# soycan-sim/bendy-tracer

Measured on AMD Instinct MI355X. Metric: Msamples/s (pixels x spp / s) at 1080p, higher is better.
Workload: dtype f32; 1 GPU; C3: scene.json.gz 1920x1080x64spp Subsample::None, Config=main.rs (max_bounces 8, max_volume_bounces 32, clip 0.01..1000, volume_step 0.1, Output::Full), flat space (the reference has no lens code), seed 0x5EED; parallelism=single

## Files before the change

### bendy_tracer_amd/api.py

```python
from __future__ import annotations

import ctypes as C
import enum
import os
from dataclasses import dataclass
from typing import Optional

import numpy as np

_HERE = os.path.dirname(os.path.abspath(__file__))
LIB_PATH = os.path.join(_HERE, "libbendy_hip.so")
BT_TILE = 16


class BendyError(RuntimeError):

    def __init__(self, code, message):
        super().__init__(f"[bt_status {code}] {message}")
        self.code = code


class Output(enum.IntEnum):
    Full = 0
    Albedo = 1
# ... 184 lines not shown


class _CLens(C.Structure):
    _fields_ = [("centre", C.c_float * 3), ("rs", C.c_float), ("step", C.c_float), ("radius", C.c_float),
                ("max_steps", C.c_uint32)]


EXPORTS = [
    "bt_config_default", "bt_render_config_default", "bt_last_error", "bt_last_error_code", "bt_version", "bt_scene_load",
    "bt_scene_from_json", "bt_scene_free", "bt_scene_find_by_tag", "bt_scene_set_camera_aspect", "bt_scene_set_lens",
    "bt_scene_object_count", "bt_scene_data_count", "bt_scene_export_prims", "bt_render", "bt_render_device",
    "bt_shard_floats", "bt_render_shard_device", "bt_unshard_device", "bt_preview_device", "bt_preview",
    "bt_comm_unique_id", "bt_comm_init", "bt_comm_free", "bt_comm_rank", "bt_comm_world", "bt_allgather_shards_device",
    "bt_exchange_frame_device", "bt_scene_last_stats", "bt_tuning_default", "bt_scene_set_tuning", "bt_scene_get_tuning", "bt_scene_default", "bt_scene_to_json", "bt_scene_save", "bt_write_png",
    "bt_scene_trim", "bt_denoise_params_default", "bt_denoiser_new", "bt_denoiser_free", "bt_denoise_device",
    "bt_denoise", "bt_debug_primary_mask", "bt_debug_block_masks_device", "bt_debug_mask_key", "bt_debug_set_object",
    "bt_debug_plan_launch",
    "bt_render_guided_device", "bt_adaptive_params_default", "bt_adaptive_new", "bt_adaptive_free", "bt_adaptive_reset",
    "bt_render_adaptive_device", "bt_adaptive_poll", "bt_adaptive_counts", "bt_adaptive_errors", "bt_debug_adaptive_moments",
    "bt_adaptive_resolve_device",
    "bt_scene_camera_view", "bt_scene_set_camera_pose", "bt_temporal_params_default", "bt_temporal_new", "bt_temporal_free",
    "bt_temporal_reset", "bt_temporal_accumulate_device", "bt_debug_temporal_history", "bt_debug_reproject",
    "bt_display_params_default", "bt_display_new", "bt_display_free", "bt_display_reset", "bt_display_device",
    "bt_display_exposure", "bt_debug_display_histogram", "bt_write_pfm", "bt_scene_export_sorted_rows",
    "bt_debug_abs_limit",
    "bt_glare_params_default", "bt_glare_new", "bt_glare_free", "bt_glare_device", "bt_debug_glare_plane", "bt_debug_glare_host",
    "bt_resample_params_default", "bt_resample_new", "bt_resample_free", "bt_resample_device", "bt_debug_resample_weights",
    "bt_debug_resample_plane", "bt_debug_resample_host",
    "bt_despeckle_params_default", "bt_despeckle_new", "bt_despeckle_free", "bt_despeckle_device", "bt_despeckle_poll",
    "bt_debug_despeckle_host",
    "bt_upscale_params_default", "bt_upscale_new", "bt_upscale_free", "bt_upscale_device", "bt_upscale_poll",
# ... 30 lines not shown
    L.bt_scene_find_by_tag.argtypes = [vp, C.c_char_p, C.POINTER(C.c_uint64)]
    L.bt_scene_set_camera_aspect.argtypes = [vp, C.c_uint64, C.c_float]
    L.bt_scene_set_lens.argtypes = [vp, C.POINTER(_CLens)]
    L.bt_scene_object_count.argtypes = [vp]
    L.bt_scene_data_count.argtypes = [vp]
    L.bt_scene_export_prims.argtypes = [vp, fp, C.c_int]
    L.bt_scene_export_sorted_rows.argtypes = [vp, C.POINTER(C.c_uint32), C.c_int]
    L.bt_debug_abs_limit.restype = C.c_float
    L.bt_debug_abs_limit.argtypes = [C.c_float]
    L.bt_debug_primary_mask.argtypes = [vp, C.c_uint64, C.POINTER(_CConfig), C.POINTER(_CRenderConfig), C.c_uint32, C.c_uint32,
                                        C.c_uint32, C.c_uint32, C.c_uint32, C.POINTER(C.c_uint64), C.c_uint32]
    L.bt_debug_set_object.argtypes = [vp, C.c_uint64, fp, C.c_float]
    L.bt_debug_block_masks_device.argtypes = L.bt_debug_primary_mask.argtypes
    L.bt_debug_mask_key.argtypes = [vp, C.c_uint64, C.POINTER(_CConfig), C.POINTER(_CRenderConfig), C.c_uint32, C.c_uint32,
                                    C.c_uint32, C.c_uint32, C.c_uint32, C.POINTER(C.c_uint8), C.c_uint32]
    L.bt_debug_plan_launch.argtypes = [vp, C.c_uint64, C.POINTER(_CConfig), C.POINTER(_CRenderConfig), C.c_uint32, C.c_uint32,
                                       C.c_uint32, C.c_uint32, C.c_int32, C.c_uint32, C.c_int32, C.c_uint32, C.c_uint64,
                                       C.POINTER(Stats)]
    L.bt_render.argtypes = [vp, C.c_uint64, C.POINTER(_CConfig), C.POINTER(_CRenderConfig), fp, C.c_uint32,
                            C.c_uint32, C.c_uint64]
    L.bt_render_device.argtypes = [vp, C.c_uint64, C.POINTER(_CConfig), C.POINTER(_CRenderConfig), vp, C.c_uint32,
                                   C.c_uint32, C.c_uint64, vp]
    L.bt_render_guided_device.argtypes = [vp, C.c_uint64, C.POINTER(_CConfig), C.POINTER(_CRenderConfig), vp, vp, vp, vp,
                                          C.c_uint32, C.c_uint32, C.c_uint64, vp]
    L.bt_shard_floats.restype = C.c_size_t
    L.bt_shard_floats.argtypes = [C.c_uint32, C.c_uint32, C.c_uint32]
    L.bt_render_shard_device.argtypes = [vp, C.c_uint64, C.POINTER(_CConfig), C.POINTER(_CRenderConfig), vp,
                                         C.c_uint32, C.c_uint32, C.c_uint32, C.c_uint32, C.c_uint64, vp]
    L.bt_unshard_device.argtypes = [vp, vp, C.c_uint32, C.c_uint32, C.c_uint32, vp]
    L.bt_preview_device.argtypes = [vp, vp, C.c_uint32, C.c_uint32, C.c_uint32, C.c_int32, vp]
# ... 410 lines not shown
                                             None, 0))
        out = np.zeros(n, dtype=np.uint64)
        _check(lib.bt_debug_primary_mask(scene._h, camera, C.byref(c), C.byref(r), width, height, slices, rank, world,
                                         out.ctypes.data_as(C.POINTER(C.c_uint64)), n))
        return out

    def block_masks_device(self, scene: Scene, camera: int, config: RenderConfig, width, height, slices, rank=0, world=1):
        c, r = _c_configs(self.config, config, 0)
        n = _check(lib.bt_debug_block_masks_device(scene._h, camera, C.byref(c), C.byref(r), width, height, slices, rank,
                                                   world, None, 0))
        out = np.zeros(n, dtype=np.uint64)
        _check(lib.bt_debug_block_masks_device(scene._h, camera, C.byref(c), C.byref(r), width, height, slices, rank, world,
                                               out.ctypes.data_as(C.POINTER(C.c_uint64)), n))
        return out

    def mask_key(self, scene: Scene, camera: int, config: RenderConfig, width, height, slices, rank=0, world=1) -> bytes:
        c, r = _c_configs(self.config, config, 0)
        n = _check(lib.bt_debug_mask_key(scene._h, camera, C.byref(c), C.byref(r), width, height, slices, rank, world, None, 0))
        out = (C.c_uint8 * n)()
        _check(lib.bt_debug_mask_key(scene._h, camera, C.byref(c), C.byref(r), width, height, slices, rank, world, out, n))
        return bytes(out)

    def plan_launch(self, scene: Scene, camera: int, config: RenderConfig, width, height, n_cu, rank=0, world=1, sharded=False,
                    kind=0, guides=0, alloc_limit=0) -> Stats:
        c, r = _c_configs(self.config, config, 0)
        st = Stats()
        _check(lib.bt_debug_plan_launch(scene._h, camera, C.byref(c), C.byref(r), width, height, rank, world, int(sharded),
                                        n_cu, kind, guides, alloc_limit, C.byref(st)))
        return st

# ... 901 lines not shown
```

### bendy_tracer_amd/csrc/bt_api.cpp

```cpp
#include <hip/hip_runtime.h>

#include <algorithm>
#include <cmath>
#include <cstdlib>
#include <cstdio>
#include <cstring>
#include <memory>
#include <string>

#include "../../include/bendy_hip.h"
#include "bt_internal.hpp"
#include "bt_scene.hpp"
#include "bt_types.h"
#include "bt_cull.hpp"
#include "bt_plan.hpp"

#pragma STDC FP_CONTRACT OFF

namespace {

thread_local std::string g_error;
thread_local int g_error_code = 0;
constexpr uint32_t kCounterSlots = 64;

// ... 39 lines not shown
    DeviceArray<BtSphereRow> d_sphere_rows;
    DeviceArray<BtRectAAN> d_aan_rows;
    DeviceArray<BtRectLA> d_la_rows;
    DeviceArray<int32_t> d_other_rows;
    DeviceArray<float> d_density;
    DeviceArray<int32_t> d_lens_prims;
    bt_lens lens_prims_for{};
    bool lens_prims_valid = false;
    unsigned long long *d_counters = nullptr;
    uint32_t render_seq = 0;
    uint32_t last_slot = 0;
    DeviceArray<float> d_scratch;
    uint32_t scratch_small_streak = 0;
    btplan::Scratch plan_scratch;
    DeviceArray<uint64_t> d_block_masks;
    btcull::MaskKey masks_for{};
    uint64_t rows_generation = 0;
    DeviceArray<float> d_host_frame;
    int n_cu = 0;
    bt_tuning tuning{};
    hipEvent_t ev_start = nullptr, ev_stop = nullptr;
    bt_stats last{};
    bool lens_on = false;
    bt_lens lens{};
    bool stats_pending = false;

    bt_scene() { bt_tuning_default(&tuning); }
    void release_device_state() {
        if (d_counters) (void)hipFree(d_counters);
        if (ev_start) (void)hipEventDestroy(ev_start);
        if (ev_stop) (void)hipEventDestroy(ev_stop);
        d_counters = nullptr;
        ev_start = ev_stop = nullptr;
        stats_pending = false;
        release_buffers();
    }
    void release_buffers() {
        d_scratch.release();
        d_host_frame.release();
        d_block_masks.release();
        masks_for = btcull::MaskKey{};
        scratch_small_streak = 0;
    }
    ~bt_scene() { release_device_state(); }
};

namespace {

int ensure_flat(bt_scene *s) {
    if (s->flat_valid) return 0;
    try {
        s->flat = bt::flatten_scene(s->scene);
    } catch (const bt::Error &e) {
        return fail(e.code, e.message);
    }
// ... 214 lines not shown
    if (!s->lens_on) return 0;
    if (!s->lens_prims_valid || std::memcmp(&s->lens_prims_for, &s->lens, sizeof(bt_lens)) != 0) {
        BT_HIP(s->d_lens_prims.upload(lens_candidates(s->flat.prims, s->lens, (double)s->lens.radius + (double)P.lens_margin)));
        s->lens_prims_for = s->lens;
        s->lens_prims_valid = true;
    }
    P.lens_prims = s->d_lens_prims.ptr;
    P.n_lens_prims = (int32_t)s->d_lens_prims.count;
    return 0;
}

int ensure_block_masks(bt_scene *s, BtLaunch &P, uint32_t n_blocks, hipStream_t stream) {
    btcull::MaskKey key;
    btcull::mask_key(key, P, n_blocks, s->rows_generation, (const void *)stream);
    if (!bt_mask_cache_enabled() || std::memcmp(&key, &s->masks_for, sizeof key) != 0) {
        if (s->d_block_masks.count < n_blocks) {
            if (s->d_block_masks.ptr) BT_HIP(hipDeviceSynchronize());
            s->masks_for = btcull::MaskKey{};
            BT_HIP(s->d_block_masks.allocate(n_blocks));
        }
        s->masks_for = btcull::MaskKey{};
        BT_HIP(bt_launch_block_masks(&P, n_blocks, s->d_block_masks.ptr, stream));
        s->masks_for = key;
    }
    P.block_masks = s->d_block_masks.ptr;
    return 0;
}

uint64_t realloc_scratch(bt_scene *s, hipStream_t stream, uint64_t need) {
    if (s->d_scratch.ptr && hipStreamSynchronize(stream) != hipSuccess) return s->d_scratch.bytes();
    s->d_scratch.release();
    if (need && s->d_scratch.allocate(need / sizeof(float)) != hipSuccess) (void)hipGetLastError();
    return s->d_scratch.bytes();
}

struct RenderPass {
    int kind = btplan::PLAIN;
    float *guides[3] = {nullptr, nullptr, nullptr};
    const uint32_t *tile_active = nullptr;
    float *moment = nullptr;
// ... 25 lines not shown
    if (rcode) return fail(rcode, plan.error);
    P.scratch = s->d_scratch.ptr;
    for (int g = 0; g < 3; ++g) {
        P.guide_out[g] = plan.output == 4 ? pass.guides[g] : nullptr;
        P.guide_scratch[g] = plan.guide_values[g] ? P.scratch + plan.guide_values[g] : nullptr;
    }
    P.tile_active = pass.tile_active;
    P.moment = pass.moment;

    s->last_slot = s->render_seq % kCounterSlots;
    if (s->last_slot == 0) BT_HIP(hipMemsetAsync(s->d_counters, 0, kCounterSlots * 16 * sizeof(unsigned long long), stream));
    s->render_seq += 1;
    P.counters = s->d_counters + (size_t)s->last_slot * 16;
    BT_HIP(hipEventRecord(s->ev_start, stream));
    P.block_masks = nullptr;
    if (bt_launch_reads_masks(&P, plan.output)) {
        rcode = ensure_block_masks(s, P, plan.grid * (uint32_t)P.slices, stream);
        if (rcode) return rcode;
    }
    {
        const uint32_t all = (uint32_t)P.samples, base = P.sample_base;
        for (uint32_t done = 0; done < all; done += plan.chunk) {
            P.samples = (int32_t)std::min(plan.chunk, all - done);
            P.sample_base = base + done;
            BT_HIP(bt_launch_render(&P, plan.output, plan.grid, plan.lds_bytes, stream));
        }
        P.samples = (int32_t)all;
        P.sample_base = base;
    }
    BT_HIP(hipEventRecord(s->ev_stop, stream));
// ... 311 lines not shown
    if (n_blocks < 0) return n_blocks;
    if (!masks || cap == 0) return n_blocks;
    if (P.any_rects || P.any_volumes) return fail(BT_ERR_INVALID_ARG, "the scene does not run the build that reads block masks");
    int rc = ensure_device(scene);
    if (rc) return rc;
    n_blocks = debug_mask_launch(scene, camera_ref, config, render, width, height, slices, rank, world, P);
    if (n_blocks < 0) return n_blocks;
    uint64_t *d = nullptr;
    BT_HIP(hipMalloc((void **)&d, sizeof(uint64_t) * (size_t)n_blocks));
    hipError_t e = bt_launch_block_masks(&P, (uint32_t)n_blocks, d, nullptr);
    if (e == hipSuccess)
        e = hipMemcpy(masks, d, sizeof(uint64_t) * (size_t)std::min<uint32_t>(cap, (uint32_t)n_blocks), hipMemcpyDeviceToHost);
    (void)hipFree(d);
    if (e != hipSuccess) return fail(BT_ERR_DEVICE, hipGetErrorString(e));
    return n_blocks;
}

int bt_debug_mask_key(bt_scene *scene, uint64_t camera_ref, const bt_config *config, const bt_render_config *render,
                      uint32_t width, uint32_t height, uint32_t slices, uint32_t rank, uint32_t world, uint8_t *out,
                      uint32_t cap) {
    BtLaunch P;
    const int n_blocks = debug_mask_launch(scene, camera_ref, config, render, width, height, slices, rank, world, P);
    if (n_blocks < 0) return n_blocks;
    btcull::MaskKey key;
    P.sphere_rows = nullptr;
    btcull::mask_key(key, P, (uint32_t)n_blocks, scene->rows_generation, nullptr);
    if (out && cap > 0) std::memcpy(out, &key, std::min<size_t>(cap, sizeof key));
    return (int)sizeof key;
}

// ... 182 lines not shown
```

### bendy_tracer_amd/csrc/bt_cull.hpp

```cpp
#pragma once
#include <stdint.h>
#include <string.h>

#include "bt_types.h"

#if defined(__HIPCC__) || defined(__HIP__)
#define BT_HD __host__ __device__ inline
#define BT_HDF static __host__ __device__ __forceinline__
#else
#define BT_HD inline
#define BT_HDF static inline
#endif

struct BlockGeom { uint32_t NS, LOG_NS, pxb, LOG_PXB, LBW, WMASK; };
BT_HDF BlockGeom block_geom(const BtLaunch &P) {
    BlockGeom g;
    g.NS = (uint32_t)P.slices;
    g.LOG_NS = (uint32_t)__builtin_ctz(g.NS);
    g.pxb = 256u >> g.LOG_NS;
    g.LOG_PXB = 8u - g.LOG_NS;
    g.LBW = g.pxb >= 32 ? 3u : 2u;
    g.WMASK = (1u << g.LBW) - 1u;
    return g;
}
// ... 186 lines not shown

template <class Rows> BT_HD uint64_t block_mask(const BtLaunch &P, Rows rows, uint32_t b) {
    const BlockGeom G = block_geom(P);
    const BlockRef B = block_ref(P, G, b);
    uint32_t nx = 0, ny = 0;
    block_extent(P, G, B, nx, ny);
    if (nx == 0u || ny == 0u || P.n_prims <= 0) return 0ull;
    if (P.n_prims > 64) return ~0ull;
    const Cone K = primary_cone(P, B.px0, B.py0, nx, ny);
    uint64_t m = 0;
    for (int i = 0; i < P.n_prims; ++i)
        if (may_hit(K, rows[i].cx, rows[i].cy, rows[i].cz, rows[i].r2)) m |= 1ull << i;
    return m;
}

struct MaskKey {
    BtV3 cam_cx, cam_cy, cam_cz, cam_t;
    float yfov, xfov, pixel_width, pixel_height;
    float jitter_u_lo, jitter_u_scale, jitter_v_lo, jitter_v_scale;
    int32_t subsample_n, has_focus;
    float focus, aperture;
    BtV3 disk_x, disk_y;
    float one_scale, clip_min;
    uint32_t width, height, tiles_x, tiles_y, tiles_x_magic;
    int32_t slices, sharded;
    uint32_t rank, world;
    int32_t n_prims;
    uint32_t n_blocks;
    uint32_t valid;
    uint64_t rows_generation;
// ... 26 lines not shown
```

### bendy_tracer_amd/csrc/bt_internal.hpp

```cpp
#pragma once
#include <hip/hip_runtime.h>

#include <string>

#include "../../include/bendy_hip.h"
#include "bt_view.hpp"

struct BtLaunch;
struct BtSphereRow;

struct BtTemporalLaunch {
    btview::View cur, prev;
    const float4 *color, *normal, *depth;
    float nc, nn, nd;
    const float4 *hist_in, *guide_in;
    float4 *hist_out, *guide_out, *out;
    float alpha_min, max_history, depth_tolerance, normal_min;
};

#define BT_DISPLAY_BINS 256
#define BT_DISPLAY_COUNTERS 258
#define BT_DISPLAY_STRIDE 260
struct BtDisplayState {
    float e;
// ... 1 lines not shown
    float shown_ev, shown_mult;
};
struct BtDisplayExpose {
    double log2_key;
    float p_low, p_high, ev, ev_min, ev_max, adapt;
};

extern "C" {
hipError_t bt_launch_render(const BtLaunch *P, int output, unsigned grid, size_t lds_bytes, hipStream_t stream);
hipError_t bt_launch_unshard(const float *gathered, float *frame, uint32_t width, uint32_t height, uint32_t tiles_x,
                             uint32_t tiles_y, uint32_t world, uint32_t tiles_per_rank, hipStream_t stream);
void bt_primary_masks_host(const BtLaunch *P, const BtSphereRow *rows, uint32_t n_blocks, uint64_t *out);
int bt_launch_reads_masks(const BtLaunch *P, int output);
int bt_mask_cache_enabled(void);
hipError_t bt_launch_block_masks(const BtLaunch *P, uint32_t n_blocks, uint64_t *masks, hipStream_t stream);
hipError_t bt_launch_preview(const float *rgba, uint8_t *out, uint32_t n, uint32_t samples, int color_space, hipStream_t stream);
hipError_t bt_launch_adapt_update(const float *rgba, const float *moment, uint32_t *count, uint32_t *active, float *error,
                                  uint32_t *n_active, uint32_t width, uint32_t height, uint32_t T, const bt_adaptive_params *p,
                                  hipStream_t stream);
hipError_t bt_launch_adapt_resolve(const float *rgba, const uint32_t *count, float *out, uint32_t width, uint32_t height,
                                   hipStream_t stream);
hipError_t bt_launch_denoise(const float *color, float nc, const float *albedo, float na, const float *normal, float nn,
                             const float *depth, float nd, float *out, float *e0, float *e1, float *guide, uint32_t width,
                             uint32_t height, uint32_t levels, float sigma_color, float sigma_normal, float sigma_depth,
                             float eps_albedo, hipStream_t stream);
hipError_t bt_launch_temporal(const BtTemporalLaunch *P, int mode, hipStream_t stream);
hipError_t bt_launch_display_meter(const float *rgba, uint64_t n, uint32_t samples, uint32_t *live, hipStream_t stream);
hipError_t bt_launch_display_expose(uint32_t *live, uint32_t *last, BtDisplayState *state, const BtDisplayExpose *p,
                                    hipStream_t stream);
hipError_t bt_launch_display_show(const float *rgba, uint8_t *out, uint64_t n, uint32_t samples, int color_space, int op,
// ... 16 lines not shown
```

### bendy_tracer_amd/csrc/bt_kernels.hip

```cpp
#include "bt_device.hpp"
#include "bt_color.hpp"
#include "bt_cull.hpp"
#include "bt_internal.hpp"

#define BT_SUM_BATCH 8

#ifdef BT_LANESTAT
#define BT_LS(i, mask) do { ls_acc[i] += (unsigned long long)__popcll(mask); } while (0)
#else
#define BT_LS(i, mask)
#endif
#ifdef BT_PROFILE
#define BT_PROF_DECL unsigned long long prof_t = __builtin_readcyclecounter(), prof_acc[BT_N_COUNTERS - 2] = {}
#define BT_PROF(i) do { const unsigned long long now_ = __builtin_readcyclecounter(); prof_acc[i] += now_ - prof_t; prof_t = now_; } while (0)
#else
#define BT_PROF_DECL
#define BT_PROF(i)
#endif

namespace {

struct Parked { float x, y, z; };
struct Parked1 { float x; };
BT_DEV V3 v3_of(const Parked &v) { return mk(v.x, v.y, v.z); }
// ... 125 lines not shown
#pragma unroll
            for (int u = 0; u < BT_SUM_BATCH; ++u) v[u] = s[(size_t)(kk + u) << g.LOG_PXB];
#pragma unroll
            for (int u = 0; u < BT_SUM_BATCH; ++u) sum = sum + v3_of(v[u]);
        }
        for (; kk < T; ++kk) {
            const PK v = s[(size_t)kk << g.LOG_PXB];
            sum = sum + v3_of(v);
        }
        o[0] = sum.x;
        o[1] = sum.y;
        o[2] = sum.z;
    }
}

template <int OUTPUT> BT_DEV void fill_empty_block(const BtLaunch &P) {
    const BlockGeom G = block_geom(P);
    const BlockRef B_own = block_ref(P, G, blockIdx.x);
    const uint32_t T = (uint32_t)P.samples * (uint32_t)(P.subsample_n * P.subsample_n);
    uint32_t nx = 0, ny = 0;
    block_extent(P, G, B_own, nx, ny);
    V3 value;
    if (OUTPUT == 0) {
        value = mk(0, 0, 0) + mk(1, 1, 1) * mk(P.root_color);
    } else if (OUTPUT == 1) {
        value = mk(P.root_albedo);
    } else {
        const float fd = P.root_has_albedo ? P.clip_max : __builtin_inff();
        float depth = (fd - P.clip_min) / (P.clip_max - P.clip_min);
        depth = fminf(fmaxf(depth, 0.0f), 1.0f);
        value = mk(depth, depth, depth);
    }
    for (uint32_t q = threadIdx.x; q < G.pxb; q += blockDim.x) {
        const PixelRef r = pixel_of(P, G, B_own, q);
        if (!r.in_frame) continue;
        float *o = out_of(P, P.out, B_own, r);
        V3 sum = mk(o[0], o[1], o[2]);
        for (uint32_t k = 0; k < T; ++k) sum = sum + value;
        o[0] = sum.x;
        o[1] = sum.y;
        o[2] = sum.z;
    }
    if (P.counters && threadIdx.x == 0 && nx * ny != 0u) atomicAdd(&P.counters[0], (unsigned long long)(nx * ny) * T);
}

}

__global__ __launch_bounds__(256) void bt_block_mask_kernel(BtLaunch P, uint32_t n_blocks, unsigned long long *masks) {
    const uint32_t b = blockIdx.x * blockDim.x + threadIdx.x;
    if (b >= n_blocks) return;
    typedef const __attribute__((address_space(4))) BtSphereRow RowK;
    masks[b] = btcull::block_mask(P, (RowK *)P.sphere_rows, b);
}

#ifndef BT_WAVES_PER_SIMD
#define BT_WAVES_PER_SIMD 7
#endif
#ifndef BT_WAVES_PER_SIMD_VOLS
#define BT_WAVES_PER_SIMD_VOLS BT_WAVES_PER_SIMD
#endif
#ifndef BT_WAVES_PER_SIMD_RECTS
#define BT_WAVES_PER_SIMD_RECTS 7
#endif
#ifndef BT_WAVES_PER_SIMD_LENS
#define BT_WAVES_PER_SIMD_LENS 6
#endif
#ifndef BT_WAVES_PER_SIMD_GUIDED_RECTS
// ... 7 lines not shown
#endif
template <int OUTPUT, bool LENS, bool RECTS, bool VOLS, bool PACKED>
__global__ __launch_bounds__(256, (OUTPUT == 4 && RECTS && !VOLS) ? BT_WAVES_PER_SIMD_GUIDED_RECTS : LENS ? BT_WAVES_PER_SIMD_LENS : (RECTS ? BT_WAVES_PER_SIMD_RECTS : (VOLS ? BT_WAVES_PER_SIMD_VOLS : BT_WAVES_PER_SIMD))) void bt_render_kernel(BtLaunch P) {
    constexpr bool GUIDED = OUTPUT == 4;
    constexpr bool ADAPT = OUTPUT == 5;
    constexpr bool AOV = OUTPUT != 0 && !ADAPT;
    constexpr bool CULL = !LENS && !RECTS && !VOLS && !PACKED && OUTPUT != 2 && !GUIDED && !ADAPT;
    if (ADAPT) {
        typedef const __attribute__((address_space(4))) BtLaunch BtLaunchK;
        typedef const __attribute__((address_space(4))) uint32_t ActiveK;
        BtLaunchK *C = (BtLaunchK *)__builtin_amdgcn_kernarg_segment_ptr();
        asm volatile("" : "+s"(C));
        const uint32_t slot = blockIdx.x >> (uint32_t)__builtin_ctz((uint32_t)C->slices);
        if (((ActiveK *)C->tile_active)[slot] == 0u) return;
    }
    if (CULL && P.max_bounces >= 0) {
        typedef const __attribute__((address_space(4))) unsigned long long MaskK;
        if (((MaskK *)P.block_masks)[blockIdx.x] == 0ull) {
            typedef const __attribute__((address_space(4))) BtLaunch BtLaunchK;
            BtLaunchK *C = (BtLaunchK *)__builtin_amdgcn_kernarg_segment_ptr();
            asm volatile("" : "+s"(C));
            fill_empty_block<OUTPUT>(*(const BtLaunch *)C);
            return;
        }
    }
    extern __shared__ __align__(16) unsigned char smem[];
    __shared__ uint32_t s_waves_done;
    __shared__ uint32_t s_next_item;
    __shared__ uint32_t s_segments;
    __shared__ uint32_t s_pool_paths[2], s_pool_waves[2];
    if (threadIdx.x == 0) {
        s_waves_done = 0;
        s_next_item = 0;
        s_segments = 0;
        if (PACKED && RECTS && !VOLS && OUTPUT == 0) s_pool_paths[0] = s_pool_paths[1] = s_pool_waves[0] = s_pool_waves[1] = 0;
    }

    SceneLds S;
    {
// ... 42 lines not shown
            bx.pad0 = bx.pad1 = 0.0f;
            vbox[i] = bx;
        }
        __syncthreads();
    }

    const BlockGeom G = block_geom(P);
    const uint32_t pxb = G.pxb, LOG_PXB = G.LOG_PXB;
    const uint32_t lane = threadIdx.x & 63;
    const uint32_t nn = (uint32_t)(P.subsample_n * P.subsample_n);
    const uint32_t T = (uint32_t)P.samples * nn;
    const uint32_t sample0 = P.sample_base * nn;
    constexpr bool packed = PACKED;
    const uint32_t my_blocks = packed ? P.wg_blocks - (blockIdx.x < P.wg_blocks_rem ? 0u : 1u) : 1u;
    const uint32_t n_items = packed ? (my_blocks << (P.log_rows + LOG_PXB)) : pxb * T;
    const BlockRef B_own = block_ref(P, G, blockIdx.x);
    auto park = [&]() -> Parked * {
        return (Parked *)P.scratch + (size_t)blockIdx.x * (packed ? (size_t)P.wg_blocks << (P.log_rows + LOG_PXB) : (size_t)n_items);
    };

    uint32_t px = 0, py = 0, pixel_index = 0, park_i = 0;

    V3 ro = mk(0, 0, 0), rd = mk(0, 0, -1), beta = mk(1, 1, 1), L = mk(0, 0, 0);
    V3 first = mk(0, 0, 0);
    float first_depth = __builtin_inff();
    bool have_first = false;
    int bounce = 0, vbounce = 0, last_object = -1;
    uint32_t event = 0;
    bool pending = true;
    constexpr bool VOTE = !RECTS && !LENS;
    bool held = false;
    float held_t = 0.0f;
    int held_info = 0, waited = 0;
    uint32_t segments = 0;
    unsigned long long lens_steps = 0;
    LensState lens;
    bool bent = false;
    lens_begin(P, lens);

    auto park_guides = [&](const V3 &albedo, const V3 &nrm, float first_t) {
        typedef const __attribute__((address_space(4))) BtLaunch BtLaunchK;
        BtLaunchK *C = (BtLaunchK *)__builtin_amdgcn_kernarg_segment_ptr();
        asm volatile("" : "+s"(C));
        const size_t at = (size_t)blockIdx.x * (packed ? (size_t)P.wg_blocks << (P.log_rows + LOG_PXB) : (size_t)n_items) + park_i;
        if (C->guide_out[0]) ((Parked *)C->guide_scratch[0])[at] = Parked{albedo.x, albedo.y, albedo.z};
        if (C->guide_out[1]) ((Parked *)C->guide_scratch[1])[at] = Parked{nrm.x, nrm.y, nrm.z};
        if (C->guide_out[2]) {
            float depth = (first_t - P.clip_min) / (P.clip_max - P.clip_min);
            depth = fminf(fmaxf(depth, 0.0f), 1.0f);
            ((Parked1 *)C->guide_scratch[2])[at] = Parked1{depth};
        }
    };
    auto park_guide_defaults = [&]() { park_guides(mk(0, 0, 0), mk(0, 0, 0), __builtin_inff()); };
    auto finish_sample = [&]() {
        V3 value;
        if (OUTPUT == 0 || GUIDED || ADAPT) {
            value = L;
        } else if (OUTPUT == 3) {
            float depth = (first_depth - P.clip_min) / (P.clip_max - P.clip_min);
// ... 455 lines not shown
    } else {
        __builtin_amdgcn_fence(__ATOMIC_RELEASE, "workgroup");
        uint32_t arrived = 0;
        if (lane == 0) arrived = atomicAdd(&s_waves_done, 1u);
        arrived = (uint32_t)__builtin_amdgcn_readfirstlane((int)arrived);
        if (arrived == (blockDim.x >> 6) - 1u) {
            __builtin_amdgcn_fence(__ATOMIC_ACQUIRE, "workgroup");
            if (P.counters && lane == 0) {
                const uint32_t total = *(volatile uint32_t *)&s_segments;
                if (total) atomicAdd(&P.counters[0], (unsigned long long)total);
            }
            if constexpr (ADAPT) {
                typedef const __attribute__((address_space(4))) BtLaunch BtLaunchK;
                BtLaunchK *C = (BtLaunchK *)__builtin_amdgcn_kernarg_segment_ptr();
                asm volatile("" : "+s"(C));
                sum_block<Parked, true>(P, G, blockIdx.x, T, park(), lane, P.out, C->moment);
            } else {
                sum_block(P, G, blockIdx.x, T, park(), lane, P.out);
            }
            if (GUIDED) {
                const size_t at = (size_t)blockIdx.x * (size_t)n_items;
                if (P.guide_out[0]) sum_block(P, G, blockIdx.x, T, (const Parked *)P.guide_scratch[0] + at, lane, P.guide_out[0]);
                if (P.guide_out[1]) sum_block(P, G, blockIdx.x, T, (const Parked *)P.guide_scratch[1] + at, lane, P.guide_out[1]);
                if (P.guide_out[2]) sum_block(P, G, blockIdx.x, T, (const Parked1 *)P.guide_scratch[2] + at, lane, P.guide_out[2]);
            }
        }
    }
    if (P.counters) {
        if (LENS) {
            unsigned long long ls = wave_sum(lens_steps);
            if (lane == 0 && ls) atomicAdd(&P.counters[1], ls);
        }
#ifdef BT_LANESTAT
        for (int i = 0; i < 9; ++i) {
            unsigned long long v = ls_acc[i];
            for (int off = 32; off > 0; off >>= 1) {
                const unsigned long long o = __shfl_xor(v, off, 64);
                v = o > v ? o : v;
            }
// ... 41 lines not shown
    return !P->any_rects && !P->any_volumes && !P->lens_on && P->wg_blocks <= 1 && output != 2 && output != 4 && output != 5 && P->max_bounces >= 0;
}
extern "C" int bt_mask_cache_enabled(void) {
#ifdef BT_MASK_NOCACHE
    return 0;
#else
    return 1;
#endif
}
extern "C" hipError_t bt_launch_block_masks(const BtLaunch *P, uint32_t n_blocks, uint64_t *masks, hipStream_t stream) {
    if (n_blocks == 0 || !masks || (P->n_prims > 0 && !P->sphere_rows)) return hipErrorInvalidValue;
    hipLaunchKernelGGL(bt_block_mask_kernel, dim3((n_blocks + 255u) / 256u), dim3(256), 0, stream, *P, n_blocks,
                       (unsigned long long *)masks);
    return hipGetLastError();
}
extern "C" hipError_t bt_launch_render(const BtLaunch *P, int output, unsigned grid, size_t lds_bytes,
                                       hipStream_t stream) {
    const bool packed = P->wg_blocks > 1;
    if (packed && P->lens_on) return hipErrorInvalidValue;
    if (bt_launch_reads_masks(P, output) && !P->block_masks) return hipErrorInvalidValue;
    dim3 g(packed ? P->n_workgroups : grid * (unsigned)P->slices), b(256);
    const int cls = (P->any_rects ? 2 : 0) | (P->any_volumes ? 1 : 0);
#define BT_LAUNCH(O, L, R, V, K)                                                                                 \
    do {                                                                                                         \
        if (lds_bytes > 48 * 1024)                                                                               \
            (void)hipFuncSetAttribute((const void *)bt_render_kernel<O, L, R, V, K>,                             \
                                      hipFuncAttributeMaxDynamicSharedMemorySize, (int)lds_bytes);               \
        hipLaunchKernelGGL((bt_render_kernel<O, L, R, V, K>), g, b, lds_bytes, stream, *P);                      \
    } while (0)
#define BT_LAUNCH_OUT(L, R, V, K)                                                                                \
    switch (output) {                                                                                            \
    case 0: BT_LAUNCH(0, L, R, V, K); break;                                                                     \
    case 1: BT_LAUNCH(1, L, R, V, K); break;                                                                     \
    case 2: BT_LAUNCH(2, L, R, V, K); break;                                                                     \
    default: BT_LAUNCH(3, L, R, V, K); break;                                                                    \
// ... 42 lines not shown
```

### bendy_tracer_amd/csrc/bt_types.h

```cpp
#pragma once
#include <stdint.h>

#define BT_TILE_DIM 16
#if defined(BT_PROFILE) || defined(BT_LANESTAT)
#define BT_N_COUNTERS 12
#else
#define BT_N_COUNTERS 2
#endif
#define BT_DENSITY_LDS_MAX 8192

struct BtV3 { float x, y, z; };

enum { BT_PRIM_SPHERE = 0, BT_PRIM_RECT = 1, BT_PRIM_RECT_AA = 2, BT_PRIM_RECT_AAN = 3, BT_PRIM_RECT_LA = 4, BT_PRIM_SHAPE_MASK = 7, BT_PRIM_STRICT = 8 };
struct BtPrim {
    int32_t kind;
    int32_t object;
    int32_t material;
    int32_t volume;
    BtV3 c;
    float radius;
    BtV3 t;
    float w_sqr;
    BtV3 icx; float h_sqr;
    BtV3 icy; int32_t aa_u;
// ... 134 lines not shown
    BtV3 lens_c;
    float lens_rs, lens_step, lens_radius;
    int32_t lens_max_steps;
    const int32_t *lens_prims;
    int32_t n_lens_prims;
    float lens_margin;
    const BtSphereRow *sphere_rows;
    uint32_t wg_blocks, wg_blocks_rem, n_workgroups;
    uint32_t pool_records, pool_lds_offset;
    uint32_t log_rows, row_mask;
    const uint64_t *block_masks;
    float *guide_out[3];
    float *guide_scratch[3];
    const uint32_t *tile_active;
    float *moment;
};
```

### include/bendy_hip.h

```cpp
#ifndef BENDY_HIP_H
#define BENDY_HIP_H

#include <stddef.h>
#include <stdint.h>

#ifdef __cplusplus
extern "C" {
#endif

typedef enum {
    BT_DONE = 0,
    BT_IN_PROGRESS = 1,
    BT_ERR_INVALID_ARG = -1,
    BT_ERR_IO = -2,
    BT_ERR_PARSE = -3,
    BT_ERR_INVALID_REF = -4,
    BT_ERR_NOT_CAMERA = -5,
    BT_ERR_NOT_MATERIAL = -6,
    BT_ERR_NO_LIGHT = -7,
    BT_ERR_DEVICE = -8,
    BT_ERR_UNSUPPORTED = -9
} bt_status;

typedef enum { BT_OUTPUT_FULL = 0, BT_OUTPUT_ALBEDO = 1, BT_OUTPUT_NORMAL = 2, BT_OUTPUT_DEPTH = 3 } bt_output;
// ... 74 lines not shown
int bt_scene_set_camera_aspect(bt_scene *scene, uint64_t camera_ref, float aspect_ratio);
int bt_scene_set_lens(bt_scene *scene, const bt_lens *lens);
int bt_scene_object_count(const bt_scene *scene);
int bt_scene_data_count(const bt_scene *scene);
int bt_scene_export_prims(const bt_scene *scene, float *out, int cap);
int bt_scene_export_sorted_rows(const bt_scene *scene, uint32_t *out, int cap);
float bt_debug_abs_limit(float limit);
int bt_debug_primary_mask(bt_scene *scene, uint64_t camera_ref, const bt_config *config, const bt_render_config *render,
                          uint32_t width, uint32_t height, uint32_t slices, uint32_t rank, uint32_t world, uint64_t *masks,
                          uint32_t cap);

int bt_debug_set_object(bt_scene *scene, uint64_t object_ref, const float *translation, float radius);
int bt_debug_block_masks_device(bt_scene *scene, uint64_t camera_ref, const bt_config *config, const bt_render_config *render,
                                uint32_t width, uint32_t height, uint32_t slices, uint32_t rank, uint32_t world,
                                uint64_t *masks, uint32_t cap);
int bt_debug_mask_key(bt_scene *scene, uint64_t camera_ref, const bt_config *config, const bt_render_config *render,
                      uint32_t width, uint32_t height, uint32_t slices, uint32_t rank, uint32_t world, uint8_t *out,
                      uint32_t cap);

int bt_debug_plan_launch(bt_scene *scene, uint64_t camera_ref, const bt_config *config, const bt_render_config *render,
                         uint32_t width, uint32_t height, uint32_t rank, uint32_t world, int32_t sharded, uint32_t n_cu,
                         int32_t pass_kind, uint32_t guides, uint64_t alloc_limit, bt_stats *out);


int bt_render(bt_scene *scene, uint64_t camera_ref, const bt_config *config, const bt_render_config *render,
              float *rgba_host, uint32_t width, uint32_t height, uint64_t seed);

int bt_render_device(bt_scene *scene, uint64_t camera_ref, const bt_config *config, const bt_render_config *render,
                     float *rgba_device, uint32_t width, uint32_t height, uint64_t seed, void *stream);

// ... 262 lines not shown
```

Before: 58050 Msamples/s.

## Compact live blocks first and batch-fill empty blocks in the render kernel

Measured after the change: 63060 Msamples/s, median of 6. +8.6%, better.

```diff
diff --git a/bendy_tracer_amd/api.py b/bendy_tracer_amd/api.py
--- a/bendy_tracer_amd/api.py
+++ b/bendy_tracer_amd/api.py
@@ -222,7 +222,7 @@
     "bt_comm_unique_id", "bt_comm_init", "bt_comm_free", "bt_comm_rank", "bt_comm_world", "bt_allgather_shards_device",
     "bt_exchange_frame_device", "bt_scene_last_stats", "bt_tuning_default", "bt_scene_set_tuning", "bt_scene_get_tuning", "bt_scene_default", "bt_scene_to_json", "bt_scene_save", "bt_write_png",
     "bt_scene_trim", "bt_denoise_params_default", "bt_denoiser_new", "bt_denoiser_free", "bt_denoise_device",
-    "bt_denoise", "bt_debug_primary_mask", "bt_debug_block_masks_device", "bt_debug_mask_key", "bt_debug_set_object",
+    "bt_denoise", "bt_debug_primary_mask", "bt_debug_block_masks_device", "bt_debug_mask_key", "bt_debug_block_order", "bt_debug_block_order_device", "bt_debug_set_object",
     "bt_debug_plan_launch",
     "bt_render_guided_device", "bt_adaptive_params_default", "bt_adaptive_new", "bt_adaptive_free", "bt_adaptive_reset",
     "bt_render_adaptive_device", "bt_adaptive_poll", "bt_adaptive_counts", "bt_adaptive_errors", "bt_debug_adaptive_moments",
@@ -283,6 +283,8 @@
     L.bt_debug_block_masks_device.argtypes = L.bt_debug_primary_mask.argtypes
     L.bt_debug_mask_key.argtypes = [vp, C.c_uint64, C.POINTER(_CConfig), C.POINTER(_CRenderConfig), C.c_uint32, C.c_uint32,
                                     C.c_uint32, C.c_uint32, C.c_uint32, C.POINTER(C.c_uint8), C.c_uint32]
+    L.bt_debug_block_order.argtypes = [C.POINTER(C.c_uint64), C.c_uint32, C.POINTER(C.c_uint32), C.POINTER(C.c_uint32)]
+    L.bt_debug_block_order_device.argtypes = L.bt_debug_block_order.argtypes
     L.bt_debug_plan_launch.argtypes = [vp, C.c_uint64, C.POINTER(_CConfig), C.POINTER(_CRenderConfig), C.c_uint32, C.c_uint32,
                                        C.c_uint32, C.c_uint32, C.c_int32, C.c_uint32, C.c_int32, C.c_uint32, C.c_uint64,
                                        C.POINTER(Stats)]
@@ -723,6 +725,15 @@
                                                out.ctypes.data_as(C.POINTER(C.c_uint64)), n))
         return out
 
+    @staticmethod
+    def block_order(masks, device=False):
+        m = np.ascontiguousarray(masks, dtype=np.uint64)
+        order, header = np.zeros(m.size, dtype=np.uint32), np.zeros(2, dtype=np.uint32)
+        fn = lib.bt_debug_block_order_device if device else lib.bt_debug_block_order
+        _check(fn(m.ctypes.data_as(C.POINTER(C.c_uint64)), m.size, order.ctypes.data_as(C.POINTER(C.c_uint32)),
+                  header.ctypes.data_as(C.POINTER(C.c_uint32))))
+        return order, (int(header[0]), int(header[1]))
+
     def mask_key(self, scene: Scene, camera: int, config: RenderConfig, width, height, slices, rank=0, world=1) -> bytes:
         c, r = _c_configs(self.config, config, 0)
         n = _check(lib.bt_debug_mask_key(scene._h, camera, C.byref(c), C.byref(r), width, height, slices, rank, world, None, 0))
diff --git a/bendy_tracer_amd/csrc/bt_api.cpp b/bendy_tracer_amd/csrc/bt_api.cpp
--- a/bendy_tracer_amd/csrc/bt_api.cpp
+++ b/bendy_tracer_amd/csrc/bt_api.cpp
@@ -77,6 +77,7 @@
     uint32_t scratch_small_streak = 0;
     btplan::Scratch plan_scratch;
     DeviceArray<uint64_t> d_block_masks;
+    DeviceArray<uint32_t> d_block_order;
     btcull::MaskKey masks_for{};
     uint64_t rows_generation = 0;
     DeviceArray<float> d_host_frame;
@@ -102,6 +103,7 @@
         d_scratch.release();
         d_host_frame.release();
         d_block_masks.release();
+        d_block_order.release();
         masks_for = btcull::MaskKey{};
         scratch_small_streak = 0;
     }
@@ -346,16 +348,19 @@
     btcull::MaskKey key;
     btcull::mask_key(key, P, n_blocks, s->rows_generation, (const void *)stream);
     if (!bt_mask_cache_enabled() || std::memcmp(&key, &s->masks_for, sizeof key) != 0) {
-        if (s->d_block_masks.count < n_blocks) {
+        if (s->d_block_masks.count < n_blocks || s->d_block_order.count < (size_t)n_blocks + BT_ORDER_HEADER) {
             if (s->d_block_masks.ptr) BT_HIP(hipDeviceSynchronize());
             s->masks_for = btcull::MaskKey{};
             BT_HIP(s->d_block_masks.allocate(n_blocks));
+            BT_HIP(s->d_block_order.allocate((size_t)n_blocks + BT_ORDER_HEADER));
         }
         s->masks_for = btcull::MaskKey{};
         BT_HIP(bt_launch_block_masks(&P, n_blocks, s->d_block_masks.ptr, stream));
+        BT_HIP(bt_launch_block_order(s->d_block_masks.ptr, n_blocks, s->d_block_order.ptr, stream));
         s->masks_for = key;
     }
     P.block_masks = s->d_block_masks.ptr;
+    P.block_order = s->d_block_order.ptr;
     return 0;
 }
 
@@ -411,6 +416,7 @@
     P.counters = s->d_counters + (size_t)s->last_slot * 16;
     BT_HIP(hipEventRecord(s->ev_start, stream));
     P.block_masks = nullptr;
+    P.block_order = nullptr;
     if (bt_launch_reads_masks(&P, plan.output)) {
         rcode = ensure_block_masks(s, P, plan.grid * (uint32_t)P.slices, stream);
         if (rcode) return rcode;
@@ -752,6 +758,28 @@
     (void)hipFree(d);
     if (e != hipSuccess) return fail(BT_ERR_DEVICE, hipGetErrorString(e));
     return n_blocks;
+}
+
+int bt_debug_block_order(const uint64_t *masks, uint32_t n_blocks, uint32_t *order_out, uint32_t *header_out) {
+    if (!masks || !order_out || !header_out || n_blocks == 0 || n_blocks > 0x7fffffffu) return fail(BT_ERR_INVALID_ARG, "bt_debug_block_order: null argument or no blocks");
+    btcull::block_order(masks, n_blocks, order_out, header_out);
+    return 0;
+}
+
+int bt_debug_block_order_device(const uint64_t *masks, uint32_t n_blocks, uint32_t *order_out, uint32_t *header_out) {
+    if (!masks || !order_out || !header_out || n_blocks == 0 || n_blocks > 0x7fffffffu) return fail(BT_ERR_INVALID_ARG, "bt_debug_block_order_device: null argument or no blocks");
+    uint64_t *d_masks = nullptr;
+    uint32_t *d_out = nullptr;
+    hipError_t e = hipMalloc((void **)&d_masks, sizeof(uint64_t) * (size_t)n_blocks);
+    if (e == hipSuccess) e = hipMalloc((void **)&d_out, sizeof(uint32_t) * ((size_t)n_blocks + BT_ORDER_HEADER));
+    if (e == hipSuccess) e = hipMemcpy(d_masks, masks, sizeof(uint64_t) * (size_t)n_blocks, hipMemcpyHostToDevice);
+    if (e == hipSuccess) e = bt_launch_block_order(d_masks, n_blocks, d_out, nullptr);
+    if (e == hipSuccess) e = hipMemcpy(header_out, d_out, sizeof(uint32_t) * BT_ORDER_HEADER, hipMemcpyDeviceToHost);
+    if (e == hipSuccess) e = hipMemcpy(order_out, d_out + BT_ORDER_HEADER, sizeof(uint32_t) * (size_t)n_blocks, hipMemcpyDeviceToHost);
+    if (d_masks) (void)hipFree(d_masks);
+    if (d_out) (void)hipFree(d_out);
+    if (e != hipSuccess) return fail(BT_ERR_DEVICE, hipGetErrorString(e));
+    return 0;
 }
 
 int bt_debug_mask_key(bt_scene *scene, uint64_t camera_ref, const bt_config *config, const bt_render_config *render,
diff --git a/bendy_tracer_amd/csrc/bt_cull.hpp b/bendy_tracer_amd/csrc/bt_cull.hpp
--- a/bendy_tracer_amd/csrc/bt_cull.hpp
+++ b/bendy_tracer_amd/csrc/bt_cull.hpp
@@ -224,6 +224,19 @@
     return m;
 }
 
+#define BT_ORDER_HEADER 2u
+BT_HD void block_order(const uint64_t *masks, uint32_t n_blocks, uint32_t *order, uint32_t *header) {
+    uint32_t n_live = 0;
+    for (uint32_t b = 0; b < n_blocks; ++b) n_live += masks[b] != 0ull ? 1u : 0u;
+    uint32_t live = 0, empty = n_live;
+    for (uint32_t b = 0; b < n_blocks; ++b) {
+        if (masks[b] != 0ull) order[live++] = b;
+        else order[empty++] = b;
+    }
+    header[0] = n_live;
+    header[1] = n_blocks - n_live;
+}
+
 struct MaskKey {
     BtV3 cam_cx, cam_cy, cam_cz, cam_t;
     float yfov, xfov, pixel_width, pixel_height;
diff --git a/bendy_tracer_amd/csrc/bt_internal.hpp b/bendy_tracer_amd/csrc/bt_internal.hpp
--- a/bendy_tracer_amd/csrc/bt_internal.hpp
+++ b/bendy_tracer_amd/csrc/bt_internal.hpp
@@ -39,6 +39,7 @@
 int bt_launch_reads_masks(const BtLaunch *P, int output);
 int bt_mask_cache_enabled(void);
 hipError_t bt_launch_block_masks(const BtLaunch *P, uint32_t n_blocks, uint64_t *masks, hipStream_t stream);
+hipError_t bt_launch_block_order(const uint64_t *masks, uint32_t n_blocks, uint32_t *out, hipStream_t stream);
 hipError_t bt_launch_preview(const float *rgba, uint8_t *out, uint32_t n, uint32_t samples, int color_space, hipStream_t stream);
 hipError_t bt_launch_adapt_update(const float *rgba, const float *moment, uint32_t *count, uint32_t *active, float *error,
                                   uint32_t *n_active, uint32_t width, uint32_t height, uint32_t T, const bt_adaptive_params *p,
diff --git a/bendy_tracer_amd/csrc/bt_kernels.hip b/bendy_tracer_amd/csrc/bt_kernels.hip
--- a/bendy_tracer_amd/csrc/bt_kernels.hip
+++ b/bendy_tracer_amd/csrc/bt_kernels.hip
@@ -163,12 +163,9 @@
     }
 }
 
-template <int OUTPUT> BT_DEV void fill_empty_block(const BtLaunch &P) {
+template <int OUTPUT> BT_DEV void fill_empty_blocks(const BtLaunch &P, const uint32_t *empties, uint32_t first, uint32_t n_empty) {
     const BlockGeom G = block_geom(P);
-    const BlockRef B_own = block_ref(P, G, blockIdx.x);
     const uint32_t T = (uint32_t)P.samples * (uint32_t)(P.subsample_n * P.subsample_n);
-    uint32_t nx = 0, ny = 0;
-    block_extent(P, G, B_own, nx, ny);
     V3 value;
     if (OUTPUT == 0) {
         value = mk(0, 0, 0) + mk(1, 1, 1) * mk(P.root_color);
@@ -180,17 +177,40 @@
         depth = fminf(fmaxf(depth, 0.0f), 1.0f);
         value = mk(depth, depth, depth);
     }
-    for (uint32_t q = threadIdx.x; q < G.pxb; q += blockDim.x) {
-        const PixelRef r = pixel_of(P, G, B_own, q);
-        if (!r.in_frame) continue;
-        float *o = out_of(P, P.out, B_own, r);
-        V3 sum = mk(o[0], o[1], o[2]);
-        for (uint32_t k = 0; k < T; ++k) sum = sum + value;
-        o[0] = sum.x;
-        o[1] = sum.y;
-        o[2] = sum.z;
-    }
-    if (P.counters && threadIdx.x == 0 && nx * ny != 0u) atomicAdd(&P.counters[0], (unsigned long long)(nx * ny) * T);
+    const uint32_t e = first + (threadIdx.x >> G.LOG_PXB);
+    if (e < n_empty) {
+        const BlockRef B = block_ref(P, G, empties[e]);
+        const PixelRef r = pixel_of(P, G, B, threadIdx.x & (G.pxb - 1u));
+        if (r.in_frame) {
+            float *o = out_of(P, P.out, B, r);
+            V3 sum = mk(o[0], o[1], o[2]);
+            for (uint32_t k = 0; k < T; ++k) sum = sum + value;
+            o[0] = sum.x;
+            o[1] = sum.y;
+            o[2] = sum.z;
+        }
+    }
+    if (P.counters && threadIdx.x < 64u) {
+        uint32_t pixels = 0;
+        if (threadIdx.x < G.NS && first + threadIdx.x < n_empty) {
+            const BlockRef B = block_ref(P, G, empties[first + threadIdx.x]);
+            uint32_t nx = 0, ny = 0;
+            block_extent(P, G, B, nx, ny);
+            pixels = nx * ny;
+        }
+#pragma unroll
+        for (int off = 32; off > 0; off >>= 1) pixels += __shfl_xor(pixels, off, 64);
+        if (threadIdx.x == 0 && pixels != 0u) atomicAdd(&P.counters[0], (unsigned long long)pixels * T);
+    }
+}
+
+BT_DEV uint32_t wave_scan_incl(uint32_t v, uint32_t lane) {
+#pragma unroll
+    for (int off = 1; off < 64; off <<= 1) {
+        const uint32_t o = __shfl_up(v, off, 64);
+        if ((int)lane >= off) v += o;
+    }
+    return v;
 }
 
 }
@@ -200,6 +220,55 @@
     if (b >= n_blocks) return;
     typedef const __attribute__((address_space(4))) BtSphereRow RowK;
     masks[b] = btcull::block_mask(P, (RowK *)P.sphere_rows, b);
+}
+
+#define BT_ORDER_THREADS 1024
+#define BT_ORDER_PER_THREAD 4
+#define BT_ORDER_CHUNK (BT_ORDER_THREADS * BT_ORDER_PER_THREAD)
+__global__ __launch_bounds__(BT_ORDER_THREADS) void bt_block_order_kernel(const unsigned long long *masks, uint32_t n_blocks, uint32_t *out) {
+    constexpr uint32_t NW = BT_ORDER_THREADS / 64;
+    __shared__ uint32_t s_wave[2][NW];
+    const uint32_t t = threadIdx.x, lane = t & 63u, wave = t >> 6;
+    uint32_t mine = 0;
+    for (uint32_t b = t; b < n_blocks; b += BT_ORDER_THREADS) mine += masks[b] != 0ull ? 1u : 0u;
+    uint32_t incl = wave_scan_incl(mine, lane);
+    if (lane == 63u) s_wave[0][wave] = incl;
+    __syncthreads();
+    uint32_t n_live = 0;
+    for (uint32_t w = 0; w < NW; ++w) n_live += s_wave[0][w];
+    if (t == 0) {
+        out[0] = n_live;
+        out[1] = n_blocks - n_live;
+    }
+    uint32_t *order = out + BT_ORDER_HEADER;
+    uint32_t live_base = 0, set = 1;
+    for (uint32_t c0 = 0; c0 < n_blocks; c0 += BT_ORDER_CHUNK, set ^= 1u) {
+        const uint32_t b0 = c0 + t * BT_ORDER_PER_THREAD;
+        bool live[BT_ORDER_PER_THREAD];
+        mine = 0;
+#pragma unroll
+        for (uint32_t j = 0; j < BT_ORDER_PER_THREAD; ++j) {
+            live[j] = b0 + j < n_blocks && masks[b0 + j] != 0ull;
+            mine += live[j] ? 1u : 0u;
+        }
+        incl = wave_scan_incl(mine, lane);
+        if (lane == 63u) s_wave[set][wave] = incl;
+        __syncthreads();
+        uint32_t before = live_base + incl - mine, total = 0;
+        for (uint32_t w = 0; w < NW; ++w) {
+            const uint32_t v = s_wave[set][w];
+            total += v;
+            if (w < wave) before += v;
+        }
+#pragma unroll
+        for (uint32_t j = 0; j < BT_ORDER_PER_THREAD; ++j) {
+            const uint32_t b = b0 + j;
+            if (b >= n_blocks) break;
+            if (live[j]) order[before++] = b;
+            else order[n_live + (b - before)] = b;
+        }
+        live_base += total;
+    }
 }
 
 #ifndef BT_WAVES_PER_SIMD
@@ -237,15 +306,22 @@
         const uint32_t slot = blockIdx.x >> (uint32_t)__builtin_ctz((uint32_t)C->slices);
         if (((ActiveK *)C->tile_active)[slot] == 0u) return;
     }
+    uint32_t bid = blockIdx.x;
     if (CULL && P.max_bounces >= 0) {
-        typedef const __attribute__((address_space(4))) unsigned long long MaskK;
-        if (((MaskK *)P.block_masks)[blockIdx.x] == 0ull) {
-            typedef const __attribute__((address_space(4))) BtLaunch BtLaunchK;
-            BtLaunchK *C = (BtLaunchK *)__builtin_amdgcn_kernarg_segment_ptr();
-            asm volatile("" : "+s"(C));
-            fill_empty_block<OUTPUT>(*(const BtLaunch *)C);
+        typedef const __attribute__((address_space(4))) BtLaunch BtLaunchK;
+        typedef const __attribute__((address_space(4))) uint32_t OrderK;
+        BtLaunchK *C = (BtLaunchK *)__builtin_amdgcn_kernarg_segment_ptr();
+        asm volatile("" : "+s"(C));
+        OrderK *ord = (OrderK *)C->block_order;
+        const uint32_t n_live = ord[0];
+        if (blockIdx.x >= n_live) {
+            const uint32_t n_empty = ord[1], log_ns = (uint32_t)__builtin_ctz((uint32_t)C->slices);
+            const uint32_t fw = blockIdx.x - n_live;
+            if (fw >= (n_empty + (1u << log_ns) - 1u) >> log_ns) return;
+            fill_empty_blocks<OUTPUT>(*(const BtLaunch *)C, (const uint32_t *)C->block_order + BT_ORDER_HEADER + n_live, fw << log_ns, n_empty);
             return;
         }
+        bid = ord[BT_ORDER_HEADER + blockIdx.x];
     }
     extern __shared__ __align__(16) unsigned char smem[];
     __shared__ uint32_t s_waves_done;
@@ -318,9 +394,9 @@
     constexpr bool packed = PACKED;
     const uint32_t my_blocks = packed ? P.wg_blocks - (blockIdx.x < P.wg_blocks_rem ? 0u : 1u) : 1u;
     const uint32_t n_items = packed ? (my_blocks << (P.log_rows + LOG_PXB)) : pxb * T;
-    const BlockRef B_own = block_ref(P, G, blockIdx.x);
+    const BlockRef B_own = block_ref(P, G, bid);
     auto park = [&]() -> Parked * {
-        return (Parked *)P.scratch + (size_t)blockIdx.x * (packed ? (size_t)P.wg_blocks << (P.log_rows + LOG_PXB) : (size_t)n_items);
+        return (Parked *)P.scratch + (size_t)bid * (packed ? (size_t)P.wg_blocks << (P.log_rows + LOG_PXB) : (size_t)n_items);
     };
 
     uint32_t px = 0, py = 0, pixel_index = 0, park_i = 0;
@@ -346,7 +422,7 @@
         typedef const __attribute__((address_space(4))) BtLaunch BtLaunchK;
         BtLaunchK *C = (BtLaunchK *)__builtin_amdgcn_kernarg_segment_ptr();
         asm volatile("" : "+s"(C));
-        const size_t at = (size_t)blockIdx.x * (packed ? (size_t)P.wg_blocks << (P.log_rows + LOG_PXB) : (size_t)n_items) + park_i;
+        const size_t at = (size_t)bid * (packed ? (size_t)P.wg_blocks << (P.log_rows + LOG_PXB) : (size_t)n_items) + park_i;
         if (C->guide_out[0]) ((Parked *)C->guide_scratch[0])[at] = Parked{albedo.x, albedo.y, albedo.z};
         if (C->guide_out[1]) ((Parked *)C->guide_scratch[1])[at] = Parked{nrm.x, nrm.y, nrm.z};
         if (C->guide_out[2]) {
@@ -832,15 +908,15 @@
                 typedef const __attribute__((address_space(4))) BtLaunch BtLaunchK;
                 BtLaunchK *C = (BtLaunchK *)__builtin_amdgcn_kernarg_segment_ptr();
                 asm volatile("" : "+s"(C));
-                sum_block<Parked, true>(P, G, blockIdx.x, T, park(), lane, P.out, C->moment);
+                sum_block<Parked, true>(P, G, bid, T, park(), lane, P.out, C->moment);
             } else {
-                sum_block(P, G, blockIdx.x, T, park(), lane, P.out);
+                sum_block(P, G, bid, T, park(), lane, P.out);
             }
             if (GUIDED) {
-                const size_t at = (size_t)blockIdx.x * (size_t)n_items;
-                if (P.guide_out[0]) sum_block(P, G, blockIdx.x, T, (const Parked *)P.guide_scratch[0] + at, lane, P.guide_out[0]);
-                if (P.guide_out[1]) sum_block(P, G, blockIdx.x, T, (const Parked *)P.guide_scratch[1] + at, lane, P.guide_out[1]);
-                if (P.guide_out[2]) sum_block(P, G, blockIdx.x, T, (const Parked1 *)P.guide_scratch[2] + at, lane, P.guide_out[2]);
+                const size_t at = (size_t)bid * (size_t)n_items;
+                if (P.guide_out[0]) sum_block(P, G, bid, T, (const Parked *)P.guide_scratch[0] + at, lane, P.guide_out[0]);
+                if (P.guide_out[1]) sum_block(P, G, bid, T, (const Parked *)P.guide_scratch[1] + at, lane, P.guide_out[1]);
+                if (P.guide_out[2]) sum_block(P, G, bid, T, (const Parked1 *)P.guide_scratch[2] + at, lane, P.guide_out[2]);
             }
         }
     }
@@ -912,11 +988,17 @@
                        (unsigned long long *)masks);
     return hipGetLastError();
 }
+extern "C" hipError_t bt_launch_block_order(const uint64_t *masks, uint32_t n_blocks, uint32_t *out, hipStream_t stream) {
+    if (n_blocks == 0 || !masks || !out) return hipErrorInvalidValue;
+    hipLaunchKernelGGL(bt_block_order_kernel, dim3(1), dim3(BT_ORDER_THREADS), 0, stream, (const unsigned long long *)masks,
+                       n_blocks, out);
+    return hipGetLastError();
+}
 extern "C" hipError_t bt_launch_render(const BtLaunch *P, int output, unsigned grid, size_t lds_bytes,
                                        hipStream_t stream) {
     const bool packed = P->wg_blocks > 1;
     if (packed && P->lens_on) return hipErrorInvalidValue;
-    if (bt_launch_reads_masks(P, output) && !P->block_masks) return hipErrorInvalidValue;
+    if (bt_launch_reads_masks(P, output) && (!P->block_masks || !P->block_order)) return hipErrorInvalidValue;
     dim3 g(packed ? P->n_workgroups : grid * (unsigned)P->slices), b(256);
     const int cls = (P->any_rects ? 2 : 0) | (P->any_volumes ? 1 : 0);
 #define BT_LAUNCH(O, L, R, V, K)                                                                                 \
diff --git a/bendy_tracer_amd/csrc/bt_types.h b/bendy_tracer_amd/csrc/bt_types.h
--- a/bendy_tracer_amd/csrc/bt_types.h
+++ b/bendy_tracer_amd/csrc/bt_types.h
@@ -172,4 +172,5 @@
     float *guide_scratch[3];
     const uint32_t *tile_active;
     float *moment;
+    const uint32_t *block_order;
 };
diff --git a/include/bendy_hip.h b/include/bendy_hip.h
--- a/include/bendy_hip.h
+++ b/include/bendy_hip.h
@@ -112,6 +112,8 @@
 int bt_debug_block_masks_device(bt_scene *scene, uint64_t camera_ref, const bt_config *config, const bt_render_config *render,
                                 uint32_t width, uint32_t height, uint32_t slices, uint32_t rank, uint32_t world,
                                 uint64_t *masks, uint32_t cap);
+int bt_debug_block_order(const uint64_t *masks, uint32_t n_blocks, uint32_t *order_out, uint32_t *header_out);
+int bt_debug_block_order_device(const uint64_t *masks, uint32_t n_blocks, uint32_t *order_out, uint32_t *header_out);
 int bt_debug_mask_key(bt_scene *scene, uint64_t camera_ref, const bt_config *config, const bt_render_config *render,
                       uint32_t width, uint32_t height, uint32_t slices, uint32_t rank, uint32_t world, uint8_t *out,
                       uint32_t cap);
diff --git a/profiles/r14/dump_compare.py b/profiles/r14/dump_compare.py
--- /dev/null
+++ b/profiles/r14/dump_compare.py
@@ -0,0 +1,9 @@
+import hashlib, os, sys
+O = sys.argv[1]
+for wl in ("c3", "c5"):
+    for f in ("frame.npy", "frame_index.npy"):
+        p = [os.path.join(O, f"dump_{wl}_{v}", f) for v in ("parent", "new")]
+        if not all(os.path.exists(q) for q in p):
+            continue
+        h = [hashlib.sha256(open(q, "rb").read()).hexdigest() for q in p]
+        print(wl, f, os.path.getsize(p[0]), "bytes", "sha256", h[0][:16], h[1][:16], "IDENTICAL" if h[0] == h[1] else "DIFFERENT")
diff --git a/profiles/r14/time_depth.py b/profiles/r14/time_depth.py
--- /dev/null
+++ b/profiles/r14/time_depth.py
@@ -0,0 +1,30 @@
+import json, os, sys
+root = os.path.abspath(sys.argv[1])
+sys.path.insert(0, root); sys.path.insert(0, os.path.join(root, "tests"))
+import numpy as np, torch
+import bendy_tracer_amd as b
+from sphere_scenes import sphere_scene
+def full_doc():
+    doc = json.loads(sphere_scene(4242, n_spheres=1, focus=False))
+    for o in doc["objects"]["collection"].values():
+        t = o["transform"]
+        for name in ("transform_world", "transform_local"):
+            if o["tag"] == "camera":
+                t[name][:9] = [1.0, 0, 0, 0, 1.0, 0, 0, 0, 1.0]; t[name][9:12] = [0.0, 0.0, 0.0]
+            else:
+                t[name][9:12] = [0.0, 0.0, -30.0]
+        if o["tag"] != "camera":
+            o["inner"]["Sphere"]["radius"] = 29.0
+    return json.dumps(doc)
+w, h, spp = 1920, 1080, 64
+out = {"tree": sys.argv[1]}
+for name, sc in (("scene.json", b.Scene.load(os.path.join(root, "scenes", "scene.json.gz"))), ("no_empty_block", b.Scene.from_json(full_doc()))):
+    cam = sc.find_by_tag("camera"); sc.set_camera_aspect(cam, w / h)
+    for output in (3, 0):
+        tr = b.Tracer.with_config(b.Config(chunks_x=8, chunks_y=4, output=b.Output(output))); rc = b.RenderConfig.with_samples(spp)
+        buf = b.Buffer.new(w, h); ms = []
+        for i in range(16):
+            tr.render(sc, cam, rc, buf, seed=0x5EED, sample_base=i * spp); torch.cuda.synchronize()
+            ms.append(sc.last_stats().kernel_ms)
+        out[f"{name}:output{output}"] = {"kernel_ms_median": round(float(np.median(ms[2:])), 4), "min": round(min(ms[2:]), 4), "max": round(max(ms[2:]), 4)}
+print(json.dumps(out))
diff --git a/profiles/r14/time_empty_frame.py b/profiles/r14/time_empty_frame.py
--- /dev/null
+++ b/profiles/r14/time_empty_frame.py
@@ -0,0 +1,26 @@
+import json, os, sys
+root = os.path.abspath(sys.argv[1])
+sys.path.insert(0, root); sys.path.insert(0, os.path.join(root, "tests"))
+import numpy as np, torch
+import bendy_tracer_amd as b
+from sphere_scenes import sphere_scene
+doc = json.loads(sphere_scene(4242, n_spheres=1, focus=False))
+for o in doc["objects"]["collection"].values():
+    t = o["transform"]
+    for name in ("transform_world", "transform_local"):
+        if o["tag"] == "camera":
+            t[name][:9] = [1.0, 0, 0, 0, 1.0, 0, 0, 0, 1.0]; t[name][9:12] = [0.0, 0.0, 0.0]
+        else:
+            t[name][9:12] = [0.0, 0.0, 6.0]
+    if o["tag"] != "camera":
+        o["inner"]["Sphere"]["radius"] = 0.5
+w, h, spp = 1920, 1080, 64
+sc = b.Scene.from_json(json.dumps(doc)); cam = sc.find_by_tag("camera"); sc.set_camera_aspect(cam, w / h)
+tr = b.Tracer.with_config(b.Config(chunks_x=8, chunks_y=4)); rc = b.RenderConfig.with_samples(spp)
+buf = b.Buffer.new(w, h); ms = []
+for i in range(int(sys.argv[2]) if len(sys.argv) > 2 else 12):
+    tr.render(sc, cam, rc, buf, seed=0x5EED, sample_base=i * spp); torch.cuda.synchronize()
+    st = sc.last_stats(); ms.append(round(st.kernel_ms, 4))
+m = tr.primary_masks(sc, cam, rc, w, h, st.slices)
+print(json.dumps({"tree": sys.argv[1], "frame": [w, h, spp], "slices": st.slices, "packed": st.packed, "blocks": int(m.size), "all_masks_zero": bool((m == 0).all()),
+                  "segments": st.segments, "kernel_ms": ms, "kernel_ms_median_after_first": float(np.median(ms[1:]))}))
```
